# DHDev0/Stochastic-muzero

Measured on NVIDIA B200. Metric: mcts_simulations_per_sec, higher is better.
Workload: dtype bf16

## Files before the change

stochastic-muzero_b200/csrc/smz_api.cu:

```cuda
#include <cuda_runtime.h>
#include <math.h>
#include <stdarg.h>
#include <stdio.h>
#include <stdlib.h>
#include <string.h>

#include <vector>

#include "../../include/smz.h"
#include "smz_kernels.h"
#include "smz_net_bf16.h"
#include "smz_net_tc32.h"
#include "smz_net_vision.h"

static thread_local char g_err[512] = "";

static int fail(int code, const char* fmt, ...) {
  va_list ap;
  va_start(ap, fmt);
  vsnprintf(g_err, sizeof(g_err), fmt, ap);
  va_end(ap);
  return code;
}

// ... 98 lines not shown
    if (c.action_dim != c.chance_dim) return fail(SMZ_E_INVALID_ARG, "smz_create: vision family needs chance_dim == action_dim");
  } else if (c.net_mode != SMZ_NET_EXTERNAL) {
    if (c.obs_dim < 1 || c.state_dim < 2 || c.hidden_dim < 1 || c.num_hidden_layers < 0)
      return fail(SMZ_E_INVALID_ARG, "smz_create: model shape out of range");
    if (c.hidden_dim > SMZ_HP || c.state_dim > SMZ_SP || c.obs_dim > SMZ_HP)
      return fail(SMZ_E_CAPACITY, "smz_create: fused MLP tiles hold H<=%d, S<=%d, obs<=%d (got %d, %d, %d)",
                  SMZ_HP, SMZ_SP, SMZ_HP, c.hidden_dim, c.state_dim, c.obs_dim);
  }
  int need = pow2ceil(c.action_dim > c.chance_dim ? c.action_dim : c.chance_dim);
  if (need < 2) need = 2;
  int lanes = c.lanes_per_tree;
  if (lanes == 0) lanes = need < 4 ? 4 : need;
  if ((lanes & (lanes - 1)) || lanes < need || lanes > 32)
    return fail(SMZ_E_INVALID_ARG, "smz_create: lanes_per_tree must be a power of two in [%d, 32]", need);

  DeviceGuard guard_(c.device);
  if (guard_.err != cudaSuccess) return fail(SMZ_E_CUDA, "cudaSetDevice(%d) failed: %s", c.device, cudaGetErrorString(guard_.err));
  smz_engine* e = new smz_engine();
  e->cfg = c;
  memset(&e->dims, 0, sizeof(e->dims));
  memset(&e->a, 0, sizeof(e->a));
  e->img32_buf = nullptr; e->blob_buf = nullptr; e->bf16 = nullptr; e->tc32 = nullptr; e->vision = nullptr;
  e->n_trees = 0; e->sims_done = 0; e->have_weights = 0; e->launches = 0; e->launches_total = 0;
  e->use_pdl = getenv("SMZ_NO_PDL") ? 0 : 1;
  e->graph_exec = nullptr; e->graph_trees = e->graph_sims = e->graph_first = -1; e->capture_stream = nullptr;

  SmzArena& a = e->a;
  a.B = c.max_trees; a.N = c.num_simulations; a.A = c.action_dim; a.C = c.chance_dim; a.K = c.max_action_sample;
  a.Kd = a.K < a.A ? a.K : a.A;
  a.Kc = a.K < a.C ? a.K : a.C;
  a.Kmax = a.Kd > a.Kc ? a.Kd : a.Kc;
  a.M = 1 + a.A + a.N * a.Kmax;
  a.W = a.A > a.C ? a.A : a.C;
  a.Sp = c.net_mode == SMZ_NET_VISION ? SMZ_VISION_SP : SMZ_SP;
  a.path_stride = a.N + 2;
  a.n_phases = 1;
  a.rng_mode = c.rng_mode;
  a.discount = (float)c.discount;
  a.one_minus_frac_f32 = (float)(1.0 - c.root_exploration_fraction);
  a.frac = c.root_exploration_fraction;
  a.alpha = c.root_dirichlet_alpha;

  e->dims.nodes_per_tree = a.M; e->dims.max_children = a.Kmax; e->dims.policy_stride = a.W;
  e->dims.hidden_stride = a.Sp; e->dims.hidden_slots = a.N + 1; e->dims.path_stride = a.path_stride;
  e->dims.lanes_per_tree = lanes;
  e->cfg.lanes_per_tree = lanes;

  const size_t B = a.B, M = a.M;
  a.row_cap = (a.B + 511) / 512 * 512 + 512;
  a.row_top = a.row_cap;
  const size_t RC = a.row_cap;
  cudaError_t r = cudaSuccess;
#define ALLOC(ptr, n) if (r == cudaSuccess) r = dev_alloc(e, &(ptr), (n))
  ALLOC(a.stat, B * M); ALLOC(a.link, B * M); ALLOC(a.root_prior, B * a.A); ALLOC(a.minmax, B);
  ALLOC(a.ucursor, B); ALLOC(a.root_to_play, B); ALLOC(a.path, B * a.path_stride); ALLOC(a.path_len, B);
  ALLOC(a.leaf_node, B); ALLOC(a.leaf_slot, B); ALLOC(a.leaf_action, B); ALLOC(a.leaf_branch, B);
  ALLOC(a.branch_count, (size_t)(a.N + 1) * 2); ALLOC(a.rows, 2 * RC); ALLOC(a.rows4, 2 * RC); ALLOC(a.error_flag, 1);
  ALLOC(a.depth_sum, 1);
  a.xin_q = c.net_mode == SMZ_NET_TC32 ? 16 : 8;
  if (c.net_mode == SMZ_NET_BF16 || c.net_mode == SMZ_NET_TC32 || c.net_mode == SMZ_NET_F16) { ALLOC(a.xin, 2 * RC * a.xin_q); }
  if (getenv("SMZ_TREE_TIMELINE")) { ALLOC(a.dbg, 8 + 4 * ((size_t)a.N + 2)); }
  ALLOC(a.out_policy, B * a.W); ALLOC(a.out_value, B); ALLOC(a.out_reward, B); ALLOC(a.dirichlet, B * a.A);
  if (c.record) {
    ALLOC(a.rec_policy, B * a.N * a.W); ALLOC(a.rec_value, B * a.N); ALLOC(a.rec_reward, B * a.N);
    ALLOC(a.rec_branch, B * a.N); ALLOC(a.rec_root_policy, B * a.W);
  }
  ALLOC(e->pbc_dev, (size_t)a.N + 2);
  ALLOC(e->rcp64_dev, (size_t)rcp_entries(a.N));
  ALLOC(e->rcp32_dev, (size_t)rcp_entries(a.N));
  ALLOC(e->seed_dev, 2);
  ALLOC(e->sign_dev, (size_t)a.N + 2);
  if (c.net_mode == SMZ_NET_VISION) {
    ALLOC(a.hidden, (size_t)(a.N + 1) * B * a.Sp);
    e->dims.weight_blob_floats = smz_vision_blob_floats(a.A, c.state_dim, c.hidden_dim, c.num_hidden_layers);
    ALLOC(e->blob_buf, e->dims.weight_blob_floats);
  } else if (c.net_mode != SMZ_NET_EXTERNAL) {
    SmzNetShape& sh = e->shape;
    sh.obs = c.obs_dim; sh.A = a.A; sh.C = a.C; sh.S = c.state_dim; sh.H = c.hidden_dim; sh.L = c.num_hidden_layers;
    sh.OH = a.W; sh.obs_pad = (c.obs_dim + 31) / 32 * 32;
    ALLOC(a.hidden, (size_t)(a.N + 1) * B * SMZ_SP);
    ALLOC(e->img32_buf, smz_net_f32_image_floats(sh));
    e->dims.weight_blob_floats = smz_blob_floats(sh);
    ALLOC(e->blob_buf, e->dims.weight_blob_floats);
  }
#undef ALLOC
  if (r != cudaSuccess) {
    for (void* p : e->allocs) cudaFree(p);
    delete e;
    return fail(SMZ_E_CUDA, "smz_create: cudaMalloc failed: %s", cudaGetErrorString(r));
  }
  a.pbc = e->pbc_dev;
  a.rcp64 = e->rcp64_dev;
  a.rcp32 = e->rcp32_dev;
  a.seed_state = e->seed_dev;
  a.sign = e->sign_dev;
  int rc = fill_default_tables(e);
  if (rc == SMZ_OK) {
    const unsigned long long st[2] = {c.seed, c.tree_id_offset};
    if (cudaMemcpy(e->seed_dev, st, sizeof(st), cudaMemcpyHostToDevice) != cudaSuccess) rc = fail(SMZ_E_CUDA, "seed upload failed");
  }
  if (rc == SMZ_OK && a.hidden) {
    cudaMemset(a.rows, 0, 2 * RC * sizeof(int));
    cudaMemset(a.rows4, 0, 2 * RC * sizeof(int4));
    if (a.xin) cudaMemset(a.xin, 0, 2 * RC * a.xin_q * sizeof(uint4));
    cudaError_t m = cudaMemset(a.hidden, 0, (size_t)(a.N + 1) * B * a.Sp * sizeof(float));
    if (m != cudaSuccess) rc = fail(SMZ_E_CUDA, "memset: %s", cudaGetErrorString(m));
  }
  if (rc == SMZ_OK && c.net_mode == SMZ_NET_BF16) rc = smz_bf16_create(e->shape, a, &e->bf16, g_err, sizeof(g_err));
  if (rc == SMZ_OK && (c.net_mode == SMZ_NET_TC32 || c.net_mode == SMZ_NET_F16))
    rc = smz_tc32_create(e->shape, c.net_mode == SMZ_NET_F16 ? 1 : 3, &e->tc32, g_err, sizeof(g_err));
  if (rc == SMZ_OK && c.net_mode == SMZ_NET_VISION)
    rc = smz_vision_create(a.A, c.state_dim, c.hidden_dim, c.num_hidden_layers, c.max_trees, &e->vision, g_err, sizeof(g_err));
  if (rc == SMZ_OK && cudaStreamCreateWithFlags(&e->capture_stream, cudaStreamNonBlocking) != cudaSuccess)
    rc = fail(SMZ_E_CUDA, "cudaStreamCreate failed");
  if (rc != SMZ_OK) { smz_destroy(e); return rc; }
  *out = e;
  return SMZ_OK;
}

int smz_destroy(smz_engine* e) {
  if (!e) return SMZ_OK;
  DeviceGuard guard_(e->cfg.device);
  if (e->a.dbg) {
    long long t[8];
    std::vector<unsigned long long> w(4 * ((size_t)e->a.N + 2));
    if (cudaMemcpy(w.data(), e->a.dbg + 8, w.size() * sizeof(w[0]), cudaMemcpyDeviceToHost) == cudaSuccess && e->a.N >= 12) {
      double tree = 0, net = 0, g1 = 0, g2 = 0;
      int n = 0;
      for (int s = e->a.N - 11; s <= e->a.N - 2; ++s, ++n) {
        const unsigned long long *c = &w[4 * s], *nx = &w[4 * (s + 1)];
        net += (double)(c[3] - c[2]);
        g1 += (double)((long long)c[0] - (long long)c[3]);
        tree += (double)(c[1] - c[0]);
        g2 += (double)((long long)nx[2] - (long long)c[1]);
      }
      fprintf(stderr, "smz step timeline (%%globaltimer, mean of %d simulations): network step %.2f us | -> tree step %.2f us | tree step %.2f us | -> network step %.2f us\n",
              n, net / n / 1e3, g1 / n / 1e3, tree / n / 1e3, g2 / n / 1e3);
    }
    if (cudaMemcpy(t, e->a.dbg, sizeof(t), cudaMemcpyDeviceToHost) == cudaSuccess)
      fprintf(stderr, "smz tree timeline (block 0, last fused launch): expand+backup %lld cycles | descent %lld cycles = %lld levels walked by warp 0 in %lld + leaf record / row reservation %lld (path length of tree 0: %lld)\n",
              t[1] - t[0], t[2] - t[1], t[5], t[4] - t[1], t[2] - t[4], t[3]);
  }
  if (e->graph_exec) cudaGraphExecDestroy(e->graph_exec);
  if (e->capture_stream) cudaStreamDestroy(e->capture_stream);
  if (e->bf16) smz_bf16_destroy(e->bf16);
  if (e->tc32) smz_tc32_destroy(e->tc32);
  if (e->vision) smz_vision_destroy(e->vision);
  for (void* p : e->allocs) cudaFree(p);
  delete e;
  return SMZ_OK;
}

int smz_get_dims(const smz_engine* e, smz_dims* out) {
  if (!e || !out) return fail(SMZ_E_INVALID_ARG, "smz_get_dims: null argument");
  *out = e->dims;
  return SMZ_OK;
}

static void drop_graph(smz_engine* e) {
  if (e->graph_exec) { cudaGraphExecDestroy(e->graph_exec); e->graph_exec = nullptr; }
  e->graph_trees = e->graph_sims = e->graph_first = -1;
}

int smz_set_pbc_table(smz_engine* e, const double* t, int32_t n) {
  if (!e || !t) return fail(SMZ_E_INVALID_ARG, "smz_set_pbc_table: null argument");
  if (n != e->a.N + 2) return fail(SMZ_E_INVALID_ARG, "smz_set_pbc_table: need %d entries, got %d", e->a.N + 2, n);
  ON_DEVICE(e);
  CU(cudaMemcpy(e->pbc_dev, t, (size_t)n * sizeof(double), cudaMemcpyHostToDevice));
  return SMZ_OK;
}

int smz_set_player_tables(smz_engine* e, const int8_t* sign, const int32_t* to_play, int32_t n_phases) {
  if (!e || !sign || !to_play || n_phases < 1) return fail(SMZ_E_INVALID_ARG, "smz_set_player_tables: bad argument");
  ON_DEVICE(e);
  const size_t n = (size_t)n_phases * (e->a.N + 2);
  signed char* d = nullptr;
  CU(dev_alloc(e, &d, n));
  CU(cudaMemcpy(d, sign, n, cudaMemcpyHostToDevice));
  e->sign_dev = d;
  e->a.sign = d;
  e->a.n_phases = n_phases;
  e->to_play_tab.assign(to_play, to_play + n);
  drop_graph(e);
  return SMZ_OK;
}

int smz_set_weights(smz_engine* e, const float* blob, uint64_t n_floats, int32_t on_device, void* stream) {
  if (!e || !blob) return fail(SMZ_E_INVALID_ARG, "smz_set_weights: null argument");
  if (e->cfg.net_mode == SMZ_NET_EXTERNAL) return fail(SMZ_E_STATE, "smz_set_weights: engine has no internal network");
  if (n_floats != e->dims.weight_blob_floats)
    return fail(SMZ_E_INVALID_ARG, "smz_set_weights: blob has %llu floats, model shape needs %llu",
                (unsigned long long)n_floats, (unsigned long long)e->dims.weight_blob_floats);
  cudaStream_t s = (cudaStream_t)stream;
  ON_DEVICE(e);
// ... 336 lines not shown
```

stochastic-muzero_b200/csrc/smz_common.cuh:

```cuda
#pragma once
#include <cuda_runtime.h>
#include <stdint.h>

#define SMZ_BRANCH_AFTERSTATE 0
#define SMZ_BRANCH_DYNAMICS 1
#define SMZ_MAX_POLICY 32
#define SMZ_HP 128
#define SMZ_SP 64
#define SMZ_VISION_SP 160

struct SmzArena {
  int B, N, A, C, K, Kd, Kc, Kmax, M, W, Sp, path_stride, n_phases;
  int row_cap, row_top;
  int4* stat;
  int2* link;
  double* root_prior;
  float2* minmax;
  int* ucursor;
  int* root_to_play;
  int4* path;
  int* path_len;
  int* leaf_node;
  int* leaf_slot;
  int* leaf_action;
  int* leaf_branch;
  int* branch_count;
  int* rows;
  int4* rows4;
  uint4* xin;
  int xin_q;
  int* error_flag;
  unsigned long long* depth_sum;
  long long* dbg;
  float* out_policy;
  float* out_value;
  float* out_reward;
  float* hidden;
  double* dirichlet;
  float* rec_policy;
  float* rec_value;
  float* rec_reward;
  signed char* rec_branch;
  float* rec_root_policy;
  int rng_mode;
  const double* tape_u;
  int tape_stride;
  const unsigned long long* seed_state;
  const double* pbc;
  const double* rcp64;
  const float* rcp32;
  const signed char* sign;
  float discount;
  float one_minus_frac_f32;
  double frac;
  double alpha;
};

#ifdef __CUDACC__
__device__ __forceinline__ unsigned long long smz_globaltimer() {
  unsigned long long t;
  asm volatile("mov.u64 %0, %%globaltimer;" : "=l"(t));
  return t;
}
__device__ __forceinline__ void smz_stamp_min(long long* dbg, int sim, int k) {
  if (dbg && threadIdx.x == 0) atomicMin(reinterpret_cast<unsigned long long*>(dbg) + 8 + 4 * sim + k, smz_globaltimer());
}
__device__ __forceinline__ void smz_stamp_max(long long* dbg, int sim, int k) {
  if (dbg && threadIdx.x == 0) atomicMax(reinterpret_cast<unsigned long long*>(dbg) + 8 + 4 * sim + k, smz_globaltimer());
}
__device__ __forceinline__ size_t smz_row_index(const SmzArena& a, int sim, int branch, int row) {
  return (size_t)(sim & 1) * a.row_cap + (branch ? a.row_top - 1 - row : row);
}
__device__ __forceinline__ void smz_pdl_wait() { asm volatile("griddepcontrol.wait;" ::: "memory"); }
__device__ __forceinline__ void smz_pdl_launch_dependents() { asm volatile("griddepcontrol.launch_dependents;" ::: "memory"); }

template <typename... KArgs, typename... Args>
inline cudaError_t smz_launch(void (*kernel)(KArgs...), dim3 grid, dim3 block, size_t smem, cudaStream_t s, bool pdl,
                              Args... args) {
  cudaLaunchConfig_t cfg{};
  cfg.gridDim = grid; cfg.blockDim = block; cfg.dynamicSmemBytes = smem; cfg.stream = s;
  cudaLaunchAttribute attr[1];
  attr[0].id = cudaLaunchAttributeProgrammaticStreamSerialization;
  attr[0].val.programmaticStreamSerializationAllowed = 1;
  cfg.attrs = attr; cfg.numAttrs = pdl ? 1 : 0;
  return cudaLaunchKernelEx(&cfg, kernel, KArgs(args)...);
}
__device__ __forceinline__ uint4 smz_philox(uint4 c, uint2 k) {
#pragma unroll
  for (int i = 0; i < 10; ++i) {
    unsigned hi0 = __umulhi(0xD2511F53u, c.x), lo0 = 0xD2511F53u * c.x;
    unsigned hi1 = __umulhi(0xCD9E8D57u, c.z), lo1 = 0xCD9E8D57u * c.z;
    c = make_uint4(hi1 ^ c.y ^ k.x, lo1, hi0 ^ c.w ^ k.y, lo0);
    k.x += 0x9E3779B9u;
    k.y += 0xBB67AE85u;
  }
  return c;
}

__device__ __forceinline__ double smz_philox_uniform(unsigned long long seed, unsigned long long tree,
                                                     unsigned index, unsigned stream) {
  uint4 r = smz_philox(make_uint4(index >> 1, stream, (unsigned)tree, (unsigned)(tree >> 32)),
                       make_uint2((unsigned)seed, (unsigned)(seed >> 32)));
  unsigned a = (index & 1) ? r.z : r.x, b = (index & 1) ? r.w : r.y;
  return ((double)(a >> 5) * 67108864.0 + (double)(b >> 6)) * (1.0 / 9007199254740992.0);
}

struct SmzRng {
  int mode, stride;
  const double* tape;
// ... 32 lines not shown
```

stochastic-muzero_b200/csrc/smz_tree.cu:

```cuda
#include <stdlib.h>

#include "smz_common.cuh"
#include "smz_kernels.h"
#include "smz_tree_dev.cuh"

namespace {

using namespace smz_tree_dev;

template <int G>
__global__ void k_root_expand(SmzArena a, int n_trees, const float* __restrict__ policy, int pstride,
                              const int* __restrict__ root_to_play, int train,
                              const double* __restrict__ dirichlet) {
  Group<G> g;
  int tree = (blockIdx.x * blockDim.x + threadIdx.x) / G;
  const bool alive = tree < n_trees;
  if (!alive) tree = n_trees - 1;
  const size_t tb = (size_t)tree * a.M;
  const int n = a.A;
  int cursor = 0;
  const float pol = (g.gl < n) ? policy[(size_t)tree * pstride + g.gl] : 0.f;
  const float p = normalise_policy(g, pol, n);
  const SmzRng rng = smz_make_rng(a);
  choice_without_replacement(g, a, rng, alive, tree, p, n, n, cursor);
// ... 49 lines not shown
}

template <int G>
__global__ void k_backup_select(SmzArena a, int n_trees, int sim) {
  smz_pdl_wait();
  smz_pdl_launch_dependents();
  Group<G> g;
  int tree = (blockIdx.x * blockDim.x + threadIdx.x) / G;
  const bool alive = tree < n_trees;
  if (!alive) tree = n_trees - 1;
  const bool stamp = a.dbg && blockIdx.x == 0 && threadIdx.x == 0;
  if (stamp) a.dbg[0] = clock64();
  const SmzRng rng = smz_make_rng(a);
  const TreeState ts = expand_backup_phase(g, a, rng, tree, alive, sim, a.out_policy, a.W, a.out_value, a.out_reward);
  __syncwarp();
  if (stamp) a.dbg[1] = clock64();
  select_phase<G>(g, a, rng, tree, alive, sim + 1, ts, nullptr, nullptr, nullptr);
  if (stamp) { a.dbg[2] = clock64(); a.dbg[3] = a.path_len[tree]; }
}

constexpr int SMZ_UWIN = 32;

__host__ __device__ inline size_t smz_mirror_bytes(int tpb, int M, int A, int n_tab, int n_pbc) {
  size_t b = (size_t)tpb * M * (sizeof(int4) + sizeof(int2));
  b += (size_t)tpb * (A + SMZ_UWIN) * sizeof(double);
  b += (size_t)(n_pbc + n_tab) * sizeof(double) + (size_t)n_tab * sizeof(float);
  return b + 16;
}

template <int G>
__global__ void k_backup_select_sm(SmzArena a, int n_trees, int sim, int n_tab) {
  extern __shared__ int4 smz_sm_nodes[];
  Group<G> g;
  int tree = (blockIdx.x * blockDim.x + threadIdx.x) / G;
  const bool alive = tree < n_trees;
  if (!alive) tree = n_trees - 1;
  const int tpb = blockDim.x / G, lt = threadIdx.x / G;
  int4* sst = smz_sm_nodes + (size_t)lt * a.M;
  int2* slk_all = reinterpret_cast<int2*>(smz_sm_nodes + (size_t)tpb * a.M);
  int2* slk = slk_all + (size_t)lt * a.M;
  double* dbl = reinterpret_cast<double*>(slk_all + (size_t)tpb * a.M + ((size_t)tpb * a.M & 1));
  double* srp = dbl + (size_t)lt * a.A;
  double* swin = dbl + (size_t)tpb * a.A + (size_t)lt * SMZ_UWIN;
  double* spbc = dbl + (size_t)tpb * (a.A + SMZ_UWIN);
  double* sr64 = spbc + (a.N + 2);
  float* sr32 = reinterpret_cast<float*>(sr64 + n_tab);

  SmzRng rng = smz_make_rng(a);
  const int cursor0 = a.ucursor[tree];
  {
    const size_t tb = (size_t)tree * a.M;
    const int used = 1 + a.A + sim * a.Kmax;
    for (int i = g.gl; i < used; i += G) {
      sst[i] = a.stat[tb + i];
      slk[i] = a.link[tb + i];
    }
    for (int i = g.gl; i < a.A; i += G) srp[i] = a.root_prior[(size_t)tree * a.A + i];
    for (int i = threadIdx.x; i < a.N + 2; i += blockDim.x) spbc[i] = a.pbc[i];
    for (int i = threadIdx.x; i < n_tab; i += blockDim.x) { sr64[i] = a.rcp64[i]; sr32[i] = a.rcp32[i]; }
    if (rng.mode == 0)
      for (int i = g.gl; i < SMZ_UWIN; i += G) swin[i] = smz_rng_uniform(rng, tree, cursor0 + i);
  }
  SmzArena al = a;
  al.pbc = spbc; al.rcp64 = sr64; al.rcp32 = sr32;
  if (rng.mode == 0) { rng.win = swin; rng.win_base = cursor0; rng.win_len = SMZ_UWIN; }
  smz_pdl_wait();
  smz_pdl_launch_dependents();
  smz_stamp_min(a.dbg, sim, 0);
  __syncthreads();
  const bool stamp = a.dbg && blockIdx.x == 0 && threadIdx.x == 0;
  if (stamp) a.dbg[0] = clock64();
  const TreeState ts = expand_backup_phase<G, true>(g, al, rng, tree, alive, sim, a.out_policy, a.W, a.out_value, a.out_reward,
                                                    sst, slk);
  __syncwarp();
  if (stamp) a.dbg[1] = clock64();
  select_phase<G, true>(g, al, rng, tree, alive, sim + 1, ts, nullptr, nullptr, nullptr, sst, slk, srp);
  if (stamp) { a.dbg[2] = clock64(); a.dbg[3] = a.path_len[tree]; }
  if (a.dbg) {
    __syncthreads();
    smz_stamp_max(a.dbg, sim, 1);
  }
}

__global__ void k_read_roots(SmzArena a, int n_trees, int* __restrict__ visits, float* __restrict__ values,
                             double* __restrict__ priors, float* __restrict__ rewards, int* __restrict__ error_out) {
  const int i = blockIdx.x * blockDim.x + threadIdx.x;
  if (i == 0 && error_out) *error_out = *a.error_flag;
  if (i >= n_trees * a.A) return;
  const int tree = i / a.A, c = i % a.A;
  const size_t tb = (size_t)tree * a.M;
  const int4 st = a.stat[tb + 1 + c];
  if (visits) visits[i] = st.x;
  if (rewards) rewards[i] = __int_as_float(st.z);
  if (priors) priors[i] = a.root_prior[i];
  if (values && c == 0) {
    const int4 r = a.stat[tb];
    values[tree] = r.x == 0 ? 0.f : __fdiv_rn(__int_as_float(r.y), (float)r.x);
  }
}

__device__ double np_sum_f64(const double* x, int n) {
  if (n < 8) {
    double r = 0.0;
    for (int i = 0; i < n; ++i) r = __dadd_rn(r, x[i]);
    return r;
  }
  double r[8];
// ... 42 lines not shown
    const double u = u_in ? u_in[tree] : smz_philox_uniform(a.seed_state[0], a.seed_state[1] + (unsigned long long)tree, 0u, 2u);
    double acc = 0.0;
    for (int i = 0; i < n; ++i) { acc = __dadd_rn(acc, p[i]); v[i] = acc; }
    for (int i = 0; i < n; ++i) pick += __ddiv_rn(v[i], acc) <= u;
    pick = pick < n ? pick : n - 1;
  } else {
    for (int i = 1; i < n; ++i) if (p[i] > p[pick]) pick = i;
  }
  if (action_out) action_out[tree] = a.link[tb + 1 + pick].y;
}

__global__ void k_dirichlet(SmzArena a, int n_trees) {
  const int tree = blockIdx.x * blockDim.x + threadIdx.x;
  if (tree >= n_trees) return;
  unsigned ctr = 0;
  const unsigned long long seed = a.seed_state[0], tid = a.seed_state[1] + (unsigned long long)tree;
  auto U = [&]() { double u = smz_philox_uniform(seed, tid, ctr++, 1u); return u > 0.0 ? u : 1.0 / 9007199254740992.0; };
  double sum = 0.0;
  for (int i = 0; i < a.A; ++i) {
    const double al = a.alpha;
    const double d = (al < 1.0 ? al + 1.0 : al) - 1.0 / 3.0, c = 1.0 / sqrt(9.0 * d);
    double gsample = d;
    for (int it = 0; it < 256; ++it) {
      const double u1 = U(), u2 = U();
      const double x = sqrt(-2.0 * log(u1)) * cospi(2.0 * u2);
      const double t = 1.0 + c * x;
      if (t <= 0.0) continue;
      const double v3 = t * t * t, u = U();
      if (log(u) < 0.5 * x * x + d - d * v3 + d * log(v3)) { gsample = d * v3; break; }
    }
    if (al < 1.0) gsample *= pow(U(), 1.0 / al);
    a.dirichlet[(size_t)tree * a.A + i] = gsample;
    sum += gsample;
  }
  for (int i = 0; i < a.A; ++i) a.dirichlet[(size_t)tree * a.A + i] /= (sum > 0.0 ? sum : 1.0);
}

template <int G>
int grid_for(int n_trees, int threads) { return (int)(((long long)n_trees * G + threads - 1) / threads); }

}

#define SMZ_DISPATCH_G(G_, CALL)        \
  switch (G_) {                         \
    case 2: { constexpr int G = 2; CALL; } break;   \
    case 4: { constexpr int G = 4; CALL; } break;   \
    case 8: { constexpr int G = 8; CALL; } break;   \
    case 16: { constexpr int G = 16; CALL; } break; \
    default: { constexpr int G = 32; CALL; } break; \
  }

static const int kThreads = 128;

void smz_launch_root_expand(const SmzArena& a, int lanes, int n_trees, const float* policy, int pstride,
                            const int* root_to_play, int train, const double* dirichlet, cudaStream_t s) {
  SMZ_DISPATCH_G(lanes, (k_root_expand<G><<<grid_for<G>(n_trees, kThreads), kThreads, 0, s>>>(
                            a, n_trees, policy, pstride, root_to_play, train, dirichlet)));
}

void smz_launch_select(const SmzArena& a, int lanes, int n_trees, int sim, int* o_slot, int* o_action, int* o_branch,
                       cudaStream_t s) {
  SMZ_DISPATCH_G(lanes, (k_select<G><<<grid_for<G>(n_trees, kThreads), kThreads, 0, s>>>(a, n_trees, sim, o_slot,
                                                                                         o_action, o_branch)));
}

void smz_launch_expand_backup(const SmzArena& a, int lanes, int n_trees, int sim, const float* policy, int pstride,
                              const float* value, const float* reward, cudaStream_t s) {
  SMZ_DISPATCH_G(lanes, (k_expand_backup<G><<<grid_for<G>(n_trees, kThreads), kThreads, 0, s>>>(
                            a, n_trees, sim, policy, pstride, value, reward)));
}

static int rcp_entries(const SmzArena& a) { return a.N + 3 > SMZ_MAX_POLICY + 1 ? a.N + 3 : SMZ_MAX_POLICY + 1; }
static size_t mirror_bytes(const SmzArena& a, int lanes) {
  return smz_mirror_bytes(kThreads / lanes, a.M, a.A, rcp_entries(a), a.N + 2);
}

bool smz_tree_mirror_fits(const SmzArena& a, int lanes) {
  const bool off = getenv("SMZ_NO_TREE_SMEM") != nullptr;
  return !off && mirror_bytes(a, lanes) <= 96 * 1024;
}

static bool mirror_pays(int blocks) {
  static int sms_of[64] = {0};
  int dev = 0;
  cudaGetDevice(&dev);
  int& sms = sms_of[dev & 63];
  if (!sms && (cudaDeviceGetAttribute(&sms, cudaDevAttrMultiProcessorCount, dev) != cudaSuccess || sms <= 0)) sms = 148;
  static const int per_sm = getenv("SMZ_MIRROR_BLOCKS_PER_SM") ? atoi(getenv("SMZ_MIRROR_BLOCKS_PER_SM")) : 2;
  return blocks <= per_sm * sms;
}

void smz_launch_backup_select(const SmzArena& a, int lanes, int n_trees, int sim, bool pdl, cudaStream_t s) {
  if (smz_tree_mirror_fits(a, lanes) && mirror_pays((n_trees * lanes + kThreads - 1) / kThreads)) {
    const size_t smem = mirror_bytes(a, lanes);
    SMZ_DISPATCH_G(lanes, (cudaFuncSetAttribute((const void*)k_backup_select_sm<G>, cudaFuncAttributeMaxDynamicSharedMemorySize,
                                                (int)smem),
                           getenv("SMZ_NO_CARVEOUT") ? cudaSuccess :
                           cudaFuncSetAttribute((const void*)k_backup_select_sm<G>, cudaFuncAttributePreferredSharedMemoryCarveout,
                                                cudaSharedmemCarveoutMaxShared),
                           smz_launch(k_backup_select_sm<G>, dim3(grid_for<G>(n_trees, kThreads)), dim3(kThreads), smem, s, pdl,
                                      a, n_trees, sim, rcp_entries(a))));
    return;
  }
  SMZ_DISPATCH_G(lanes, (smz_launch(k_backup_select<G>, dim3(grid_for<G>(n_trees, kThreads)), dim3(kThreads), 0, s, pdl,
                                    a, n_trees, sim)));
}

void smz_launch_read_roots(const SmzArena& a, int n_trees, int* visits, float* values, double* priors, float* rewards,
                           int* error_out, cudaStream_t s) {
  const int n = n_trees * a.A;
  k_read_roots<<<(n + 255) / 256, 256, 0, s>>>(a, n_trees, visits, values, priors, rewards, error_out);
}

void smz_launch_select_actions(const SmzArena& a, int n_trees, double temperature, const double* u, int* actions,
                               double* policy, double* stored, cudaStream_t s) {
  k_select_actions<<<(n_trees + 127) / 128, 128, 0, s>>>(a, n_trees, temperature, u, actions, policy, stored);
}

__global__ void k_begin_search(SmzArena a) {
  for (int i = threadIdx.x; i < (a.N + 1) * 2; i += blockDim.x) a.branch_count[i] = 0;
  if (threadIdx.x == 0) { *a.error_flag = 0; *a.depth_sum = 0ull; }
}
void smz_launch_begin_search(const SmzArena& a, cudaStream_t s) { k_begin_search<<<1, 128, 0, s>>>(a); }

__global__ void k_set_seed(unsigned long long* dst, unsigned long long seed, unsigned long long tree_id_offset) {
  dst[0] = seed;
  dst[1] = tree_id_offset;
}
void smz_launch_set_seed(unsigned long long* dst, unsigned long long seed, unsigned long long tree_id_offset, cudaStream_t s) {
  k_set_seed<<<1, 1, 0, s>>>(dst, seed, tree_id_offset);
}

void smz_launch_dirichlet(const SmzArena& a, int n_trees, cudaStream_t s) {
  k_dirichlet<<<(n_trees + 127) / 128, 128, 0, s>>>(a, n_trees);
}
```

stochastic-muzero_b200/csrc/smz_tree_dev.cuh:

```cuda
#pragma once
#include "smz_common.cuh"

namespace smz_tree_dev {

#define FULL 0xffffffffu

template <int G>
struct Group {
  int lane, gl, gbase;
  __device__ Group() {
    lane = threadIdx.x & 31;
    gl = lane & (G - 1);
    gbase = lane & ~(G - 1);
  }
  template <typename T>
  __device__ T bcast(T v, int src) const { return __shfl_sync(FULL, v, src, G); }
  __device__ unsigned ballot(bool p) const {
    unsigned b = __ballot_sync(FULL, p);
    return (G == 32) ? b : ((b >> gbase) & ((1u << G) - 1u));
  }
};

template <int G>
__device__ float np_sum_f32(const Group<G>& g, float a, int n) {
// ... 15 lines not shown
      const float v = g.bcast(a, (i + j) & (G - 1));
      if (i < nb) r[j] = __fadd_rn(r[j], v);
    }
  }
  float res = __fadd_rn(__fadd_rn(__fadd_rn(r[0], r[1]), __fadd_rn(r[2], r[3])),
                        __fadd_rn(__fadd_rn(r[4], r[5]), __fadd_rn(r[6], r[7])));
#pragma unroll
  for (int t = 0; t < 7; ++t) {
    const float v = g.bcast(a, (nb + t) & (G - 1));
    if (nb + t < n) res = __fadd_rn(res, v);
  }
  return n < 8 ? seq : res;
}

template <int G>
__device__ double choice_cdf_raw(const Group<G>& g, double p, int n, double& total) {
  double acc = 0.0, mine = 0.0;
  if constexpr (G >= 16) {
    double sc = p;
    bool inexact = false;
#pragma unroll
    for (int off = 1; off < G; off <<= 1) {
      const double o = __shfl_up_sync(FULL, sc, off, G);
      if (g.gl >= off) {
        const double t = __dadd_rn(sc, o);
        const double bv = __dsub_rn(t, sc);
        const double err = __dadd_rn(__dsub_rn(sc, __dsub_rn(t, bv)), __dsub_rn(o, bv));
        inexact |= err != 0.0;
        sc = t;
      }
    }
    if (!__any_sync(FULL, inexact)) {
      total = g.bcast(sc, G - 1);
      return sc;
    }
  }
#pragma unroll
  for (int i = 0; i < G; ++i) {
    acc = __dadd_rn(acc, g.bcast(p, i));
    if (g.gl == i) mine = acc;
  }
  total = acc;
  return mine;
}
constexpr float SMZ_CDF_MARGIN = 2e-6f;
__device__ __forceinline__ float cdf_f32(double num, double total, bool in_range) {
  return in_range ? __fdividef((float)num, (float)total) : 3.f;
}
__device__ __forceinline__ double cdf_exact(double num, double total, bool in_range) {
  return in_range ? __ddiv_rn(num, total) : 2.0;
}

template <int G>
__device__ int searchsorted_right(const Group<G>& g, double num, double total, int n, double u) {
  const float cf = cdf_f32(num, total, g.gl < n), uf = (float)u;
  int cnt = 0;
  bool close = false;
  if constexpr (G >= 16) {
#pragma unroll
    for (int step = G / 2; step >= 1; step >>= 1) {
      const float cv = g.bcast(cf, cnt + step - 1);
      close |= fabsf(cv - uf) <= SMZ_CDF_MARGIN;
      if (cv < uf) cnt += step;
    }
  } else {
#pragma unroll
    for (int i = 0; i < G; ++i) {
      const float cv = g.bcast(cf, i);
      close |= fabsf(cv - uf) <= SMZ_CDF_MARGIN;
      cnt += cv < uf;
    }
  }
  if (__any_sync(FULL, close)) {
    const double c = cdf_exact(num, total, g.gl < n);
    cnt = 0;
    if constexpr (G >= 16) {
#pragma unroll
      for (int step = G / 2; step >= 1; step >>= 1) {
        const double cv = g.bcast(c, cnt + step - 1);
        if (cv <= u) cnt += step;
      }
    } else {
#pragma unroll
      for (int i = 0; i < G; ++i) cnt += g.bcast(c, i) <= u;
    }
  }
  return cnt;
}

template <int G>
__device__ float normalise_policy(const Group<G>& g, float pol, int n) {
  const float p = (g.gl < n) ? __fadd_rn(pol, 1e-12f) : 0.f;
  const float s = np_sum_f32(g, p, n);
  return (g.gl < n) ? __fdiv_rn(p, s) : 0.f;
}

template <int G>
__device__ unsigned choice_without_replacement(const Group<G>& g, const SmzArena& a, const SmzRng& rng, bool alive, int tree,
                                               float p32, int n, int bound, int& cursor) {
  unsigned found = 0;
  int nf = alive ? 0 : bound;
  if (g.ballot(alive && g.gl < n && !(p32 >= 0.f))) {
    if (alive) *a.error_flag = 2;
    found = bound >= 32 ? 0xffffffffu : ((1u << bound) - 1u);
    nf = bound;
  }
  const double pd = (g.gl < n) ? (double)p32 : 0.0;
  for (int round = 0; __any_sync(FULL, nf < bound); ++round) {
    if (round > 2 * SMZ_MAX_POLICY) {
      if (nf < bound) {
        *a.error_flag = 2;
        for (int i = 0; i < n && nf < bound; ++i)
          if (!((found >> i) & 1u)) { found |= 1u << i; ++nf; }
      }
      break;
    }
    const int m = bound - nf;
    double total;
    const double num = choice_cdf_raw(g, ((found >> g.gl) & 1u) ? 0.0 : pd, n, total);
    const bool on = g.gl < m;
    double u = 2.0;
    if (__any_sync(FULL, on)) {
      if (on) u = smz_rng_uniform(rng, tree, cursor + g.gl);
    }
    const int cnt = searchsorted_right(g, num, total, n, u);
    const int idx = cnt < n ? cnt : n - 1;
    unsigned bits = on ? (1u << idx) : 0u;
#pragma unroll
    for (int off = G / 2; off > 0; off >>= 1) bits |= __shfl_xor_sync(FULL, bits, off, G);
    found |= bits;
    nf = alive ? __popc(found) : bound;
    cursor += m;
  }
  return found;
}


struct TreeState {
  int cursor;
  float2 mm;
  int2 root;
};

template <int G, bool MIRROR = false>
__device__ __forceinline__ void select_phase(const Group<G>& g, const SmzArena& a, const SmzRng& rng, int tree, bool alive,
                                             int sim, TreeState ts, int* __restrict__ o_slot, int* __restrict__ o_action,
                                             int* __restrict__ o_branch, const int4* __restrict__ sst = nullptr,
                                             const int2* __restrict__ slk = nullptr, const double* __restrict__ srp = nullptr) {
  const size_t tb = (size_t)tree * a.M;
  int cursor = ts.cursor;
  const float vmin = ts.mm.x, vmax = ts.mm.y;
  int4* path = a.path + (size_t)tree * a.path_stride;

  int depth = 0, cbase = 1, nch = a.A;
  int parent_visit = ts.root.x;
  const float range = __fsub_rn(vmax, vmin);
  const float rrange = vmax > vmin ? __frcp_rn(range) : 0.f;
  const bool range_plain = (__float_as_int(range) & 0x7FFFFF) == 0x7FFFFF || range < 1e-30f;
  if (alive && g.gl == 0) path[0] = make_int4(0, ts.root.x, ts.root.y, 0);
  int L = 1, child = 0, child_key = 0;
  bool going = alive;
  const double prior0 = (alive && g.gl < a.A) ? (srp ? srp[g.gl] : a.root_prior[(size_t)tree * a.A + g.gl]) : 0.0;
  int level = 0;
  while (__any_sync(FULL, going)) {
    const bool act = going && g.gl < nch;
    const bool chance = (level >> 1) & 1;
    const int ci = act ? cbase + g.gl : 0;
    int4 st;
    int2 lk;
    if constexpr (MIRROR) {
      st = sst[ci];
      lk = slk[ci];
    } else {
      st = a.stat[tb + ci];
      lk = a.link[tb + ci];
    }
    if (!act) { st = make_int4(0, 0, 0, 0); lk = make_int2(0, 0); }
    const double pbc = chance ? 0.0 : a.pbc[going ? parent_visit : 0];
    const int uidx = chance ? cursor : cursor + g.gl;
    const bool want = going && (chance || act);
    const unsigned wofs = (unsigned)(uidx - rng.win_base);
    const bool hit = rng.win != nullptr && wofs < (unsigned)rng.win_len;
    double u = hit ? rng.win[wofs] : 0.0;
    if (__any_sync(FULL, want && !hit)) {
      if (want && !hit) u = smz_rng_uniform(rng, tree, uidx);
    }
    int pick = 0;
    if (chance) {
      const float p = __int_as_float(st.w);
      const float om = act ? __fadd_rn(__fsub_rn(1.f, p), 1e-12f) : 0.f;
      const float rem = fabsf(smz_div_r32(np_sum_f32(g, om, nch), (float)nch, a.rcp32[nch]));
      const float sh = act ? __fadd_rn(p, rem) : 0.f;
      const float tot = np_sum_f32(g, sh, nch);
      const float q = act ? __fdiv_rn(sh, tot) : 0.f;
      double total;
      const double num = choice_cdf_raw(g, (double)q, nch, total);
      const float cf = cdf_f32(num, total, act), uf = (float)u;
      bool le = cf < uf;
      const bool close = act && fabsf(cf - uf) <= SMZ_CDF_MARGIN;
      if (__any_sync(FULL, close)) {
        if (close) le = __ddiv_rn(num, total) <= u;
      }
      int pk = __popc(g.ballot(act && le));
      pk = pk < nch ? pk : nch - 1;
      if (chance) { pick = pk; cursor += going ? 1 : 0; }
    }
    if (!chance) {
      double score = -__longlong_as_double(0x7ff0000000000000LL);
      int best = -1;
      if (act && !chance) {
        const double prior = (level == 0) ? prior0 : (double)__int_as_float(st.w);
        const double ps = smz_div_r64(__dmul_rn(pbc, prior), (double)(st.x + 1), a.rcp64[st.x + 1]);
        double vs = 0.0;
        if (st.x > 0) {
          const float val = smz_div_r32(__int_as_float(st.y), (float)st.x, a.rcp32[st.x]);
          float v = __fadd_rn(__int_as_float(st.z), __fmul_rn(a.discount, val));
          if (vmax > vmin) v = range_plain ? __fdiv_rn(__fsub_rn(v, vmin), range) : smz_div_r32(__fsub_rn(v, vmin), range, rrange);
          vs = (double)v;
        }
        const double noise = __dadd_rn(1e-7, __dmul_rn(2e-7 - 1e-7, u));
        score = __dadd_rn(__dadd_rn(ps, vs), noise);
        best = g.gl;
      }
#pragma unroll
      for (int off = G / 2; off > 0; off >>= 1) {
        const double os = __shfl_xor_sync(FULL, score, off, G);
        const int ob = __shfl_xor_sync(FULL, best, off, G);
        if (os > score || (os == score && ob > best)) { score = os; best = ob; }
      }
      if (!chance) { pick = best < 0 ? 0 : best; cursor += going ? nch : 0; }
    }
    const int4 cst = make_int4(g.bcast(st.x, pick), g.bcast(st.y, pick), g.bcast(st.z, pick), 0);
    const int child_cb = g.bcast(lk.x, pick);
    const int key = g.bcast(lk.y, pick);
    if (going) {
      child = cbase + pick;
      child_key = key;
      if (g.gl == 0) path[L] = make_int4(child, cst.x, cst.y, cst.z);
      ++L;
      if (child_cb == 0 || L >= a.path_stride) {
        going = false;
      } else {
        nch = chance ? a.Kd : a.Kc;
        parent_visit = cst.x;
        cbase = child_cb;
        ++depth;
      }
    }
    ++level;
  }
  if (a.dbg && blockIdx.x == 0 && threadIdx.x == 0) { a.dbg[4] = clock64(); a.dbg[5] = level; }
  const bool lead = alive && g.gl == 0;
  const int branch = ((depth >> 1) & 1) ? SMZ_BRANCH_DYNAMICS : SMZ_BRANCH_AFTERSTATE;
  const int slot = (cbase == 1) ? 0 : (cbase - 1 - a.A) / a.Kmax + 1;
  uint4 hcopy[(G < 8) ? 8 / G : 1], hcopy2[(G < 8) ? 8 / G : 1];
  const bool copy_row = a.xin != nullptr && alive;
  const bool wide_row = a.xin_q > 8;
  if (copy_row) {
    const uint4* src = reinterpret_cast<const uint4*>(a.hidden) + ((size_t)slot * a.B + tree) * a.xin_q;
#pragma unroll
    for (int j = 0; j < ((G < 8) ? 8 / G : 1); ++j) {
      const int idx = g.gl + j * G;
      hcopy[j] = idx < 8 ? src[idx] : make_uint4(0, 0, 0, 0);
      if (wide_row) hcopy2[j] = idx < 8 ? src[8 + idx] : make_uint4(0, 0, 0, 0);
    }
  }
  int r = 0;
  {
    const unsigned lane = threadIdx.x & 31u;
    __shared__ int s_cnt[2], s_base[2];
    if (threadIdx.x < 2) s_cnt[threadIdx.x] = 0;
    __syncthreads();
#pragma unroll
    for (int b = 0; b < 2; ++b) {
      const unsigned m = __ballot_sync(FULL, lead && branch == b);
      if (m) {
        const int leader = __ffs(m) - 1;
        int base = 0;
        if ((int)lane == leader) base = atomicAdd(&s_cnt[b], __popc(m));
        base = __shfl_sync(FULL, base, leader);
        if (lead && branch == b) r = base + __popc(m & ((1u << lane) - 1u));
      }
    }
    __syncthreads();
    if (threadIdx.x < 2) s_base[threadIdx.x] = s_cnt[threadIdx.x] ? atomicAdd(&a.branch_count[sim * 2 + threadIdx.x], s_cnt[threadIdx.x]) : 0;
    __syncthreads();
    r += s_base[branch];
  }
  const int rg = g.bcast(r, 0);
  if (copy_row) {
    uint4* dst = a.xin + smz_row_index(a, sim, branch, rg) * a.xin_q;
#pragma unroll
    for (int j = 0; j < ((G < 8) ? 8 / G : 1); ++j) {
      const int idx = g.gl + j * G;
      if (idx < 8) dst[idx] = hcopy[j];
      if (wide_row && idx < 8) dst[8 + idx] = hcopy2[j];
    }
  }
  {
    int dsum = lead ? depth + 1 : 0;
#pragma unroll
    for (int off = 16; off > 0; off >>= 1) dsum += __shfl_xor_sync(FULL, dsum, off);
    if ((threadIdx.x & 31u) == 0 && dsum) atomicAdd(a.depth_sum, (unsigned long long)dsum);
  }
  if (lead) {
    a.leaf_node[tree] = child;
    a.leaf_slot[tree] = slot;
    a.leaf_action[tree] = child_key;
    a.leaf_branch[tree] = branch;
    a.path_len[tree] = L;
    a.ucursor[tree] = cursor;
    if (o_slot) o_slot[tree] = slot;
    if (o_action) o_action[tree] = child_key;
    if (o_branch) o_branch[tree] = branch;
    a.rows[smz_row_index(a, sim, branch, r)] = tree;
    a.rows4[smz_row_index(a, sim, branch, r)] = make_int4(tree, slot, child_key, 0);
  }
}

template <int G, bool MIRROR = false>
__device__ __forceinline__ TreeState expand_backup_phase(const Group<G>& g, const SmzArena& a, const SmzRng& rng, int tree,
                                                         bool alive, int sim, const float* __restrict__ policy,
                                                         int pstride, const float* __restrict__ value,
                                                         const float* __restrict__ reward, int4* __restrict__ sst = nullptr,
                                                         int2* __restrict__ slk = nullptr) {
  const size_t tb = (size_t)tree * a.M;
  const int4* path = a.path + (size_t)tree * a.path_stride;
  const int4 rec0 = (g.gl < a.path_stride) ? path[g.gl] : make_int4(0, 0, 0, 0);
  const int4 rec1 = (G + g.gl < a.path_stride) ? path[G + g.gl] : make_int4(0, 0, 0, 0);
  const int leaf = a.leaf_node[tree];
  const int branch = a.leaf_branch[tree];
  const int L = alive ? a.path_len[tree] : 0;
  int cursor = a.ucursor[tree];
  float2 mm = a.minmax[tree];
  float v = value[tree];
  const float rew_in = reward[tree];
  const signed char* sign = a.sign + (size_t)a.root_to_play[tree] * (a.N + 2);

  const int n = branch ? a.A : a.C;
  const int bound = min(a.K, n);
  const float pol = (g.gl < n) ? policy[(size_t)tree * pstride + g.gl] : 0.f;
  const float p = normalise_policy(g, pol, n);
  const unsigned found = choice_without_replacement(g, a, rng, alive, tree, p, n, bound, cursor);
  const int cb = 1 + a.A + sim * a.Kmax;
  if (alive && g.gl < n && ((found >> g.gl) & 1u)) {
    const int r = __popc(found & ((1u << g.gl) - 1u));
    a.stat[tb + cb + r] = make_int4(0, 0, 0, __float_as_int(p));
    a.link[tb + cb + r] = make_int2(0, g.gl);
    if constexpr (MIRROR) {
      sst[cb + r] = make_int4(0, 0, 0, __float_as_int(p));
      slk[cb + r] = make_int2(0, g.gl);
    }
  }
  const float rew = branch ? rew_in : 0.f;
  if (alive && g.gl == 0) {
    a.link[tb + leaf].x = cb;
    a.ucursor[tree] = cursor;
    if (branch) reinterpret_cast<int*>(a.stat + tb + leaf)[2] = __float_as_int(rew);
    if constexpr (MIRROR) {
      slk[leaf].x = cb;
      if (branch) sst[leaf].z = __float_as_int(rew);
    }
    if (a.rec_policy) {
      const size_t ro = ((size_t)tree * a.N + sim);
      for (int i = 0; i < a.W; ++i) a.rec_policy[ro * a.W + i] = i < n ? policy[(size_t)tree * pstride + i] : 0.f;
      a.rec_value[ro] = v;
      a.rec_reward[ro] = rew;
      a.rec_branch[ro] = (signed char)branch;
    }
  }

  int2 root = make_int2(0, 0);
  int l_max = L;
#pragma unroll
  for (int off = 16; off > 0; off >>= 1) l_max = max(l_max, __shfl_xor_sync(FULL, l_max, off));
  const int n_chunks = (l_max + G - 1) / G;
  for (int chunk = n_chunks - 1; chunk >= 0; --chunk) {
    const int l = chunk * G + g.gl;
    const bool valid = l < L;
    int4 rec = chunk == 0 ? rec0 : rec1;
    if (chunk > 1 && valid) rec = path[l];
    if (!valid) rec = make_int4(0, 0, 0, 0);
    if (valid && l == L - 1 && branch) rec.w = __float_as_int(rew);
    const float r = __int_as_float(rec.w);
    float myv = 0.f;
    if constexpr (G >= 16) {
      for (int t = min(G, l_max - chunk * G) - 1; t >= 0; --t) {
        const float ri = g.bcast(r, t);
        if (chunk * G + t < L) {
          if (g.gl == t) myv = v;
          v = __fadd_rn(ri, __fmul_rn(a.discount, v));
        }
      }
    } else {
#pragma unroll
      for (int t = G - 1; t >= 0; --t) {
        const float ri = g.bcast(r, t);
        if (chunk * G + t < L) {
          if (g.gl == t) myv = v;
          v = __fadd_rn(ri, __fmul_rn(a.discount, v));
        }
      }
    }
    if (valid) {
// ... 26 lines not shown
```

Measured before the change: 186.8 million.

## Precompute chance-node CDF at expansion and reuse it during descent

Computes the chance-node cumulative distribution once, when children are expanded, and stores it in a new per-node cdf array (or in the shared mirror's w field). During selection it then reads the stored value instead of redoing the normalisation and prefix-sum reductions at every chance level, recomputing only for near-tie cases. The cost is an extra global array with its stores, a compacted child layout for wider groups, and a heuristic that disables the stored path for narrow-lane, non-mirrored configurations. It also adds per-warp, per-level clock instrumentation that is active only under a debug environment variable.

```diff
diff --git a/stochastic-muzero_b200/csrc/smz_api.cu b/stochastic-muzero_b200/csrc/smz_api.cu
--- a/stochastic-muzero_b200/csrc/smz_api.cu
+++ b/stochastic-muzero_b200/csrc/smz_api.cu
@@ -174,14 +174,14 @@
   const size_t RC = a.row_cap;
   cudaError_t r = cudaSuccess;
 #define ALLOC(ptr, n) if (r == cudaSuccess) r = dev_alloc(e, &(ptr), (n))
-  ALLOC(a.stat, B * M); ALLOC(a.link, B * M); ALLOC(a.root_prior, B * a.A); ALLOC(a.minmax, B);
+  ALLOC(a.stat, B * M); ALLOC(a.link, B * M); ALLOC(a.cdf, B * M); ALLOC(a.root_prior, B * a.A); ALLOC(a.minmax, B);
   ALLOC(a.ucursor, B); ALLOC(a.root_to_play, B); ALLOC(a.path, B * a.path_stride); ALLOC(a.path_len, B);
   ALLOC(a.leaf_node, B); ALLOC(a.leaf_slot, B); ALLOC(a.leaf_action, B); ALLOC(a.leaf_branch, B);
   ALLOC(a.branch_count, (size_t)(a.N + 1) * 2); ALLOC(a.rows, 2 * RC); ALLOC(a.rows4, 2 * RC); ALLOC(a.error_flag, 1);
   ALLOC(a.depth_sum, 1);
   a.xin_q = c.net_mode == SMZ_NET_TC32 ? 16 : 8;
   if (c.net_mode == SMZ_NET_BF16 || c.net_mode == SMZ_NET_TC32 || c.net_mode == SMZ_NET_F16) { ALLOC(a.xin, 2 * RC * a.xin_q); }
-  if (getenv("SMZ_TREE_TIMELINE")) { ALLOC(a.dbg, 8 + 4 * ((size_t)a.N + 2)); }
+  if (getenv("SMZ_TREE_TIMELINE")) { ALLOC(a.dbg, smz_dbg_words(a.N)); }
   ALLOC(a.out_policy, B * a.W); ALLOC(a.out_value, B); ALLOC(a.out_reward, B); ALLOC(a.dirichlet, B * a.A);
   if (c.record) {
     ALLOC(a.rec_policy, B * a.N * a.W); ALLOC(a.rec_value, B * a.N); ALLOC(a.rec_reward, B * a.N);
@@ -262,6 +262,28 @@
     if (cudaMemcpy(t, e->a.dbg, sizeof(t), cudaMemcpyDeviceToHost) == cudaSuccess)
       fprintf(stderr, "smz tree timeline (block 0, last fused launch): expand+backup %lld cycles | descent %lld cycles = %lld levels walked by warp 0 in %lld + leaf record / row reservation %lld (path length of tree 0: %lld)\n",
               t[1] - t[0], t[2] - t[1], t[5], t[4] - t[1], t[2] - t[4], t[3]);
+    std::vector<long long> ws((size_t)SMZ_DBG_WARPS * SMZ_DBG_WARP);
+    if (cudaMemcpy(ws.data(), e->a.dbg + smz_dbg_warp_base(e->a.N), ws.size() * sizeof(long long), cudaMemcpyDeviceToHost) == cudaSuccess) {
+      double sum[2] = {0, 0};
+      int cnt[2] = {0, 0}, deep = 0;
+      for (int w = 0; w < SMZ_DBG_WARPS; ++w) {
+        const long long* s = &ws[(size_t)w * SMZ_DBG_WARP];
+        if (s[SMZ_DBG_LV] > ws[(size_t)deep * SMZ_DBG_WARP + SMZ_DBG_LV]) deep = w;
+        for (int k = 1; k < s[SMZ_DBG_LV] && k < SMZ_DBG_LEVELS; ++k) { sum[(k >> 1) & 1] += (double)(s[1 + k] - s[k]); ++cnt[(k >> 1) & 1]; }
+      }
+      const long long* s = &ws[(size_t)deep * SMZ_DBG_WARP];
+      fprintf(stderr, "smz tree levels (block 0, last fused launch, cycles; D decision, C chance): deepest warp %d walks %lld levels:",
+              deep, s[SMZ_DBG_LV]);
+      for (int k = 0; k < s[SMZ_DBG_LV] && k < SMZ_DBG_LEVELS; ++k)
+        fprintf(stderr, " %c%lld", ((k >> 1) & 1) ? 'C' : 'D', s[1 + k] - s[k]);
+      fprintf(stderr, "\n  mean over the %d warps of block 0, levels >= 1: decision %.0f cycles (%d levels), chance %.0f cycles (%d levels)\n",
+              SMZ_DBG_WARPS, cnt[0] ? sum[0] / cnt[0] : 0.0, cnt[0], cnt[1] ? sum[1] / cnt[1] : 0.0, cnt[1]);
+      for (int w = 0; w < SMZ_DBG_WARPS; ++w) {
+        const long long* r = &ws[(size_t)w * SMZ_DBG_WARP + SMZ_DBG_SYNC0];
+        fprintf(stderr, "  leaf record, warp %d (%lld levels): wait at the first __syncthreads %lld | block ranks %lld | global row atomic round trip %lld | stores %lld\n",
+                w, ws[(size_t)w * SMZ_DBG_WARP + SMZ_DBG_LV], r[1] - r[0], r[2] - r[1], r[3] - r[2], r[4] - r[3]);
+      }
+    }
   }
   if (e->graph_exec) cudaGraphExecDestroy(e->graph_exec);
   if (e->capture_stream) cudaStreamDestroy(e->capture_stream);
diff --git a/stochastic-muzero_b200/csrc/smz_common.cuh b/stochastic-muzero_b200/csrc/smz_common.cuh
--- a/stochastic-muzero_b200/csrc/smz_common.cuh
+++ b/stochastic-muzero_b200/csrc/smz_common.cuh
@@ -14,6 +14,7 @@
   int row_cap, row_top;
   int4* stat;
   int2* link;
+  float* cdf;
   double* root_prior;
   float2* minmax;
   int* ucursor;
@@ -55,6 +56,11 @@
   double frac;
   double alpha;
 };
+
+constexpr int SMZ_DBG_LEVELS = 24, SMZ_DBG_LV = 1 + SMZ_DBG_LEVELS, SMZ_DBG_SYNC0 = SMZ_DBG_LV + 1,
+              SMZ_DBG_WARP = SMZ_DBG_SYNC0 + 5, SMZ_DBG_WARPS = 4;
+inline __host__ __device__ size_t smz_dbg_warp_base(int N) { return 8 + 4 * ((size_t)N + 2); }
+inline size_t smz_dbg_words(int N) { return smz_dbg_warp_base(N) + (size_t)SMZ_DBG_WARPS * SMZ_DBG_WARP; }
 
 #ifdef __CUDACC__
 __device__ __forceinline__ unsigned long long smz_globaltimer() {
diff --git a/stochastic-muzero_b200/csrc/smz_tree.cu b/stochastic-muzero_b200/csrc/smz_tree.cu
--- a/stochastic-muzero_b200/csrc/smz_tree.cu
+++ b/stochastic-muzero_b200/csrc/smz_tree.cu
@@ -125,7 +125,9 @@
     const size_t tb = (size_t)tree * a.M;
     const int used = 1 + a.A + sim * a.Kmax;
     for (int i = g.gl; i < used; i += G) {
-      sst[i] = a.stat[tb + i];
+      int4 st = a.stat[tb + i];
+      if (i > a.A) st.w = __float_as_int(a.cdf[tb + i]);
+      sst[i] = st;
       slk[i] = a.link[tb + i];
     }
     for (int i = g.gl; i < a.A; i += G) srp[i] = a.root_prior[(size_t)tree * a.A + i];
@@ -274,6 +276,13 @@
 
 static const int kThreads = 128;
 
+static bool mirror_pays(int blocks);
+static SmzArena with_cdf_policy(const SmzArena& a, int lanes, int n_trees) {
+  SmzArena b = a;
+  if (lanes < 16 && !mirror_pays((n_trees * lanes + kThreads - 1) / kThreads)) b.cdf = nullptr;
+  return b;
+}
+
 void smz_launch_root_expand(const SmzArena& a, int lanes, int n_trees, const float* policy, int pstride,
                             const int* root_to_play, int train, const double* dirichlet, cudaStream_t s) {
   SMZ_DISPATCH_G(lanes, (k_root_expand<G><<<grid_for<G>(n_trees, kThreads), kThreads, 0, s>>>(
@@ -282,14 +291,14 @@
 
 void smz_launch_select(const SmzArena& a, int lanes, int n_trees, int sim, int* o_slot, int* o_action, int* o_branch,
                        cudaStream_t s) {
-  SMZ_DISPATCH_G(lanes, (k_select<G><<<grid_for<G>(n_trees, kThreads), kThreads, 0, s>>>(a, n_trees, sim, o_slot,
-                                                                                         o_action, o_branch)));
+  SMZ_DISPATCH_G(lanes, (k_select<G><<<grid_for<G>(n_trees, kThreads), kThreads, 0, s>>>(with_cdf_policy(a, lanes, n_trees),
+                                                                                         n_trees, sim, o_slot, o_action, o_branch)));
 }
 
 void smz_launch_expand_backup(const SmzArena& a, int lanes, int n_trees, int sim, const float* policy, int pstride,
                               const float* value, const float* reward, cudaStream_t s) {
   SMZ_DISPATCH_G(lanes, (k_expand_backup<G><<<grid_for<G>(n_trees, kThreads), kThreads, 0, s>>>(
-                            a, n_trees, sim, policy, pstride, value, reward)));
+                            with_cdf_policy(a, lanes, n_trees), n_trees, sim, policy, pstride, value, reward)));
 }
 
 static int rcp_entries(const SmzArena& a) { return a.N + 3 > SMZ_MAX_POLICY + 1 ? a.N + 3 : SMZ_MAX_POLICY + 1; }
@@ -325,7 +334,7 @@
     return;
   }
   SMZ_DISPATCH_G(lanes, (smz_launch(k_backup_select<G>, dim3(grid_for<G>(n_trees, kThreads)), dim3(kThreads), 0, s, pdl,
-                                    a, n_trees, sim)));
+                                    with_cdf_policy(a, lanes, n_trees), n_trees, sim)));
 }
 
 void smz_launch_read_roots(const SmzArena& a, int n_trees, int* visits, float* values, double* priors, float* rewards,
diff --git a/stochastic-muzero_b200/csrc/smz_tree_dev.cuh b/stochastic-muzero_b200/csrc/smz_tree_dev.cuh
--- a/stochastic-muzero_b200/csrc/smz_tree_dev.cuh
+++ b/stochastic-muzero_b200/csrc/smz_tree_dev.cuh
@@ -91,6 +91,18 @@
 }
 
 template <int G>
+__device__ float chance_cdf(const Group<G>& g, const SmzArena& a, float p, int nch, bool act, double& num, double& total) {
+  const int ns = G < 8 ? G : nch;
+  const float om = act ? __fadd_rn(__fsub_rn(1.f, p), 1e-12f) : 0.f;
+  const float rem = fabsf(smz_div_r32(np_sum_f32(g, om, ns), (float)nch, a.rcp32[nch]));
+  const float sh = act ? __fadd_rn(p, rem) : 0.f;
+  const float tot = np_sum_f32(g, sh, ns);
+  const float q = act ? __fdiv_rn(sh, tot) : 0.f;
+  num = choice_cdf_raw(g, (double)q, nch, total);
+  return cdf_f32(num, total, act);
+}
+
+template <int G>
 __device__ int searchsorted_right(const Group<G>& g, double num, double total, int n, double u) {
   const float cf = cdf_f32(num, total, g.gl < n), uf = (float)u;
   int cnt = 0;
@@ -174,6 +186,11 @@
   return found;
 }
 
+
+__device__ __forceinline__ void tree_stamp(const SmzArena& a, int k, long long v = -1) {
+  if (a.dbg && blockIdx.x == 0 && (threadIdx.x & 31) == 0 && threadIdx.x < 32 * SMZ_DBG_WARPS)
+    a.dbg[smz_dbg_warp_base(a.N) + (threadIdx.x >> 5) * SMZ_DBG_WARP + k] = v < 0 ? clock64() : v;
+}
 
 struct TreeState {
   int cursor;
@@ -200,19 +217,24 @@
   int L = 1, child = 0, child_key = 0;
   bool going = alive;
   const double prior0 = (alive && g.gl < a.A) ? (srp ? srp[g.gl] : a.root_prior[(size_t)tree * a.A + g.gl]) : 0.0;
+  const bool stored = MIRROR || G >= 16 || a.cdf != nullptr;
   int level = 0;
+  tree_stamp(a, 0);
   while (__any_sync(FULL, going)) {
     const bool act = going && g.gl < nch;
     const bool chance = (level >> 1) & 1;
     const int ci = act ? cbase + g.gl : 0;
     int4 st;
     int2 lk;
+    float cf = 3.f;
     if constexpr (MIRROR) {
       st = sst[ci];
       lk = slk[ci];
+      cf = __int_as_float(st.w);
     } else {
       st = a.stat[tb + ci];
       lk = a.link[tb + ci];
+      if (chance && stored) cf = a.cdf[tb + ci];
     }
     if (!act) { st = make_int4(0, 0, 0, 0); lk = make_int2(0, 0); }
     const double pbc = chance ? 0.0 : a.pbc[going ? parent_visit : 0];
@@ -226,18 +248,16 @@
     }
     int pick = 0;
     if (chance) {
-      const float p = __int_as_float(st.w);
-      const float om = act ? __fadd_rn(__fsub_rn(1.f, p), 1e-12f) : 0.f;
-      const float rem = fabsf(smz_div_r32(np_sum_f32(g, om, nch), (float)nch, a.rcp32[nch]));
-      const float sh = act ? __fadd_rn(p, rem) : 0.f;
-      const float tot = np_sum_f32(g, sh, nch);
-      const float q = act ? __fdiv_rn(sh, tot) : 0.f;
-      double total;
-      const double num = choice_cdf_raw(g, (double)q, nch, total);
-      const float cf = cdf_f32(num, total, act), uf = (float)u;
+      const float uf = (float)u;
+      double num, total;
+      if (!stored) cf = chance_cdf(g, a, __int_as_float(st.w), nch, act, num, total);
       bool le = cf < uf;
       const bool close = act && fabsf(cf - uf) <= SMZ_CDF_MARGIN;
       if (__any_sync(FULL, close)) {
+        if (stored) {
+          const float p = act ? __int_as_float(reinterpret_cast<const int*>(a.stat + tb + ci)[3]) : 0.f;
+          chance_cdf(g, a, p, nch, act, num, total);
+        }
         if (close) le = __ddiv_rn(num, total) <= u;
       }
       int pk = __popc(g.ballot(act && le));
@@ -287,8 +307,10 @@
       }
     }
     ++level;
+    if (level <= SMZ_DBG_LEVELS) tree_stamp(a, level);
   }
   if (a.dbg && blockIdx.x == 0 && threadIdx.x == 0) { a.dbg[4] = clock64(); a.dbg[5] = level; }
+  tree_stamp(a, SMZ_DBG_LV, level);
   const bool lead = alive && g.gl == 0;
   const int branch = ((depth >> 1) & 1) ? SMZ_BRANCH_DYNAMICS : SMZ_BRANCH_AFTERSTATE;
   const int slot = (cbase == 1) ? 0 : (cbase - 1 - a.A) / a.Kmax + 1;
@@ -309,7 +331,9 @@
     const unsigned lane = threadIdx.x & 31u;
     __shared__ int s_cnt[2], s_base[2];
     if (threadIdx.x < 2) s_cnt[threadIdx.x] = 0;
+    tree_stamp(a, SMZ_DBG_SYNC0);
     __syncthreads();
+    tree_stamp(a, SMZ_DBG_SYNC0 + 1);
 #pragma unroll
     for (int b = 0; b < 2; ++b) {
       const unsigned m = __ballot_sync(FULL, lead && branch == b);
@@ -322,9 +346,11 @@
       }
     }
     __syncthreads();
+    tree_stamp(a, SMZ_DBG_SYNC0 + 2);
     if (threadIdx.x < 2) s_base[threadIdx.x] = s_cnt[threadIdx.x] ? atomicAdd(&a.branch_count[sim * 2 + threadIdx.x], s_cnt[threadIdx.x]) : 0;
     __syncthreads();
     r += s_base[branch];
+    tree_stamp(a, SMZ_DBG_SYNC0 + 3);
   }
   const int rg = g.bcast(r, 0);
   if (copy_row) {
@@ -355,6 +381,7 @@
     a.rows[smz_row_index(a, sim, branch, r)] = tree;
     a.rows4[smz_row_index(a, sim, branch, r)] = make_int4(tree, slot, child_key, 0);
   }
+  tree_stamp(a, SMZ_DBG_SYNC0 + 4);
 }
 
 template <int G, bool MIRROR = false>
@@ -382,13 +409,26 @@
   const float p = normalise_policy(g, pol, n);
   const unsigned found = choice_without_replacement(g, a, rng, alive, tree, p, n, bound, cursor);
   const int cb = 1 + a.A + sim * a.Kmax;
-  if (alive && g.gl < n && ((found >> g.gl) & 1u)) {
-    const int r = __popc(found & ((1u << g.gl) - 1u));
-    a.stat[tb + cb + r] = make_int4(0, 0, 0, __float_as_int(p));
-    a.link[tb + cb + r] = make_int2(0, g.gl);
+  constexpr bool kInPlace = G < 8;
+  const int nc = __popc(found);
+  const bool mine = kInPlace ? alive && g.gl < n && ((found >> g.gl) & 1u) : alive && g.gl < nc;
+  const int r = kInPlace ? __popc(found & ((1u << g.gl) - 1u)) : g.gl;
+  const int key = kInPlace ? g.gl : (mine ? __fns(found, 0, g.gl + 1) : 0);
+  const float pc = kInPlace ? p : g.bcast(p, key);
+  float w = pc;
+  const bool chance_leaf = alive && (((L - 1) >> 1) & 1);
+  if (a.cdf && __any_sync(FULL, chance_leaf)) {
+    double num, total;
+    const float cf = chance_cdf(g, a, pc, nc, chance_leaf && mine, num, total);
+    if (chance_leaf) w = cf;
+  }
+  if (mine) {
+    a.stat[tb + cb + r] = make_int4(0, 0, 0, __float_as_int(pc));
+    a.link[tb + cb + r] = make_int2(0, key);
+    if (a.cdf) a.cdf[tb + cb + r] = w;
     if constexpr (MIRROR) {
-      sst[cb + r] = make_int4(0, 0, 0, __float_as_int(p));
-      slk[cb + r] = make_int2(0, g.gl);
+      sst[cb + r] = make_int4(0, 0, 0, __float_as_int(w));
+      slk[cb + r] = make_int2(0, key);
     }
   }
   const float rew = branch ? rew_in : 0.f;
```

New measurement: 189.2 million (median of 6 runs). 1.01x the previous value.
